# neuzxy/Distributed-TF-Serving

Hardware: AMD Instinct MI355X
Metric: CTR scores/sec (whole node) (higher is better)
Workload: dtype bf16; 1 GPU; model=deepfm (1Mx64 emb, 43 fields, MLP 1024-512-256), global_batch=16384, request_rows=512, parallelism=candidate-dp1 (one GPU, no fan-out), encoding=raw, aux_lane_cus=0

## Files before the change

### csrc/bindings_hip.cpp

```cpp
#include <torch/extension.h>

#include <cstring>

#include <ATen/hip/HIPContext.h>
#include <c10/core/DeviceGuard.h>
#include <c10/hip/HIPStream.h>

#include "kernels/launchers.h"
#include "comm/rccl_comm.h"
#include "live_bindings.h"
#include "runtime/numa.h"
#include "runtime/step_runner.h"

namespace {

hipStream_t cur_stream(const torch::Tensor& t) { return c10::hip::getCurrentHIPStream(t.device().index()).stream(); }

void check_hip(hipError_t e, const char* what) {
  TORCH_CHECK(e == hipSuccess, what, " failed: ", hipGetErrorString(e));
}

void check_dev(const torch::Tensor& t, const char* name) {
  TORCH_CHECK(t.is_cuda(), name, " must be a GPU tensor");
  TORCH_CHECK(t.is_contiguous(), name, " must be contiguous");
// ... 1183 lines not shown
                  reinterpret_cast<uintptr_t>(X.data_ptr()) % 16 == 0,
              "X needs unit column stride and 16-byte aligned rows");
  TORCH_CHECK(W2p.scalar_type() == torch::kFloat8_e4m3fn && W3p.scalar_type() == torch::kFloat8_e4m3fn,
              "W2p, W3p must be e4m3 (pack_bfrag_fp8)");
  TORCH_CHECK(W2p.numel() == N2 * K1 && W3p.numel() == N3 * N2, "packed weight sizes: 512 x 1024 and 256 x 512");
  for (auto* t : {&sw2, &b2, &sw3, &b3, &hw})
    TORCH_CHECK(t->scalar_type() == torch::kFloat32, "sw2, b2, sw3, b3, hw must be fp32");
  TORCH_CHECK(sw2.numel() == N2 && b2.numel() == N2, "sw2, b2 must have 512 elements");
  TORCH_CHECK(sw3.numel() == N3 && b3.numel() == N3 && hw.numel() == N3, "sw3, b3, hw must have 256 elements");
  TORCH_CHECK((act2 == 0 || act2 == 1) && (act3 == 0 || act3 == 1), "act must be 0 (none) or 1 (relu)");
  if (extra) {
    check_gpu(*extra, "extra");
    check_same_dev(X, *extra, "extra");
    check_extra(*extra, M);
  }
  if (out && out->is_cuda()) check_same_dev(X, *out, "out");
  c10::DeviceGuard g(X.device());
  torch::Tensor y;
  float* yp = score_out(X, M, out, y);
  check_hip(dtfs::launch_mlp_tail_fp8(X.data_ptr(), M <= 1 ? K1 : X.stride(0), int(M), int(K1), W2p.data_ptr(),
                                      sw2.data_ptr<float>(), b2.data_ptr<float>(), int(act2), int(N2), W3p.data_ptr(),
                                      sw3.data_ptr<float>(), b3.data_ptr<float>(), int(act3), int(N3),
                                      hw.data_ptr<float>(), float(hbias),
                                      extra ? extra->data_ptr<float>() : nullptr, extra ? extra_rows(*extra) : 0,
                                      extra ? extra_stride(*extra) : 0, sigmoid ? 2 : 0, yp, cur_stream(X)),
            "mlp_tail_fp8");
  return y;
}

torch::Tensor gather_mlp(torch::Tensor table, c10::optional<torch::Tensor> lin, c10::optional<torch::Tensor> arena,
                         c10::optional<torch::Tensor> ids, c10::optional<torch::Tensor> wts, int64_t B, int64_t F,
                         int64_t modulo, double bias, torch::Tensor W1p, torch::Tensor b1, torch::Tensor W2p,
                         torch::Tensor b2, int64_t act2, torch::Tensor W3p, torch::Tensor b3, int64_t act3,
                         torch::Tensor hw, double hbias, bool fm, bool sigmoid, c10::optional<torch::Tensor> out) {
  check_dev(table, "table");
  for (auto* t : {&W1p, &b1, &W2p, &b2, &W3p, &b3, &hw}) {
    check_dev(*t, "gather_mlp operand");
    check_same_dev(table, *t, "gather_mlp operand");
  }
  TORCH_CHECK(table.scalar_type() == torch::kBFloat16 && table.dim() == 2 && table.size(1) == 64 &&
                  table.is_contiguous(),
              "gather_mlp: table must be contiguous bf16 [V, 64]");
  const int64_t V = table.size(0);
  TORCH_CHECK(F >= 1 && F <= 64, "gather_mlp handles 1..64 fields");
  TORCH_CHECK(modulo > 0, "modulo must be positive");
  for (auto* t : {&W1p, &W2p, &W3p})
    TORCH_CHECK(t->scalar_type() == torch::kBFloat16 && t->is_contiguous(), "W1p / W2p / W3p: contiguous bf16 (pack_frag32)");
  TORCH_CHECK(b1.scalar_type() == torch::kFloat32 && b1.numel() == 1024 && b2.scalar_type() == torch::kFloat32 &&
                  b2.numel() == 512 && b3.scalar_type() == torch::kFloat32 && b3.numel() == 256 &&
                  hw.scalar_type() == torch::kFloat32 && hw.numel() == 256,
              "gather_mlp covers 64F -> 1024 -> 512 -> 256 -> 1 (fp32 biases / head weights)");
  TORCH_CHECK(W1p.numel() == 1024 * 64 * F && W2p.numel() == 512 * 1024 && W3p.numel() == 256 * 512,
              "packed weight sizes");
  TORCH_CHECK((act2 == 0 || act2 == 1) && (act3 == 0 || act3 == 1), "act must be 0 (none) or 1 (relu)");
  TORCH_CHECK(B >= 0 && B < (int64_t(1) << 31), "gather_mlp: row count");
  if (lin) {
    check_dev(*lin, "lin");
    TORCH_CHECK(lin->scalar_type() == torch::kFloat32 && lin->numel() == V, "lin must be fp32 [V]");
  }
  TORCH_CHECK(dtfs::gather_mlp_ok((B + 63) / 64 * 64, 1024, int(64 * F), 512, 256, int(F), V),
              "gather_mlp: shape outside the kernel's range");
  dtfs::EmbedArgs a;
  embed_gemm_inputs(table, arena, ids, wts, B, F, a);
  a.table = table.data_ptr();
  a.lin = lin ? lin->data_ptr<float>() : nullptr;
  a.B = int(B);
  a.F = int(F);
  a.D = 64;
  a.V = V;
  a.modulo = modulo;
  a.bias = float(bias);
  c10::DeviceGuard g(table.device());
  torch::Tensor y;
  float* yp = score_out(table, B, out, y);
  if (B == 0) return y;
  check_hip(dtfs::launch_gather_mlp(a, W1p.data_ptr(), b1.data_ptr<float>(), W2p.data_ptr(), b2.data_ptr<float>(),
                                    int(act2), W3p.data_ptr(), b3.data_ptr<float>(), int(act3), hw.data_ptr<float>(),
                                    float(hbias), fm, sigmoid ? 2 : 0, yp, cur_stream(table)),
            "gather_mlp");
  return y;
}

void unpack_arena(torch::Tensor arena, torch::Tensor packed, int64_t fields, int64_t narrow_modulo) {
  check_dev(arena, "arena");
  check_dev(packed, "packed");
  check_same_dev(arena, packed, "packed");
  TORCH_CHECK(arena.scalar_type() == torch::kUInt8 && arena.numel() > dtfs::kArenaPayloadOff, "arena: uint8 [cap]");
  TORCH_CHECK(packed.scalar_type() == torch::kInt64 && packed.dim() == 2, "packed must be int64 [B, W]");
  TORCH_CHECK(packed.size(1) * 8 >= (narrow_modulo > 0 ? 8 : 12) * fields, "packed rows too narrow for the field count");
  TORCH_CHECK(narrow_modulo >= 0 && narrow_modulo < (int64_t(1) << 31), "narrow_modulo must fit int32 rows");
  c10::DeviceGuard g(arena.device());
  check_hip(dtfs::launch_unpack_arena(arena.data_ptr(), packed.data_ptr<int64_t>(), int(packed.size(0)), int(fields),
                                      int(packed.size(1)), dtfs::kArenaMaxRequests, cur_stream(arena), narrow_modulo),
            "unpack_arena");
}

void arena_varint_decode(torch::Tensor arena, int64_t blocks) {
  check_dev(arena, "arena");
  TORCH_CHECK(arena.scalar_type() == torch::kUInt8 && arena.numel() > dtfs::kArenaPayloadOff, "arena: uint8 [cap]");
  c10::DeviceGuard g(arena.device());
  check_hip(dtfs::launch_arena_varint(arena.data_ptr(), int(blocks), cur_stream(arena)), "arena_varint_decode");
}

void pull_host(torch::Tensor dst, torch::Tensor src, int64_t nbytes, int64_t blocks) {
  check_dev(dst, "dst");
  TORCH_CHECK(src.device().is_cpu() && src.is_pinned(), "src must be pinned host memory");
  TORCH_CHECK(nbytes >= 0 && nbytes <= dst.nbytes() && nbytes <= src.nbytes(), "nbytes out of range");
  c10::DeviceGuard g(dst.device());
  check_hip(dtfs::launch_pull_host(dst.data_ptr(), src.data_ptr(), nbytes, int(blocks), cur_stream(dst)), "pull_host");
}

// ... 627 lines not shown
        py::arg("ring") = py::none(), py::arg("ring_ctr") = py::none(), py::arg("sample_every") = 0,
        py::arg("out_cols") = 0,
        "K1 + K5 with the rows read where they live (peer stores over xGMI, replica cache first)");
  m.def("peer_bag", &peer_bag, py::arg("ids"), py::arg("wts"), py::arg("arena"), py::arg("B"), py::arg("col0"),
        py::arg("hot"), py::arg("cbase"), py::arg("towner"), py::arg("toff"), py::arg("trows"), py::arg("tremote"),
        py::arg("chunk_shift"), py::arg("cache") = py::none(), py::arg("stats") = py::none(),
        py::arg("ring") = py::none(), py::arg("ring_ctr") = py::none(), py::arg("sample_every") = 0, py::arg("out"),
        "K1b multi-hot bags with the rows read where they live -> bf16 [B, T, 64]");
  m.def("peer_cache_fill", &peer_cache_fill, py::arg("keys"), py::arg("slots"), py::arg("cbase"), py::arg("towner"),
        py::arg("toff"), py::arg("trows"), py::arg("tremote"), py::arg("chunk_shift"), py::arg("rows"),
        "replica cache: copy the keys' table rows into their slots");
  m.def("device_alloc", &device_alloc, py::arg("nbytes"), py::arg("like"),
        "uint8 device buffer of exactly nbytes (its own hipMalloc allocation)");
  m.def("cache_index_build", &cache_index_build, py::arg("keys"), py::arg("slots"), py::arg("entries"),
        "replica cache: open-addressing index keys -> slots ({key, slot} entries pre-filled with -1)");
  m.def("ipc_export", &ipc_export, py::arg("t"), "(IPC handle bytes, byte offset) of a device tensor's allocation");
  m.def("ipc_open", &ipc_open, py::arg("handle"), py::arg("offset"), py::arg("shape"), py::arg("like"),
        "map a peer's ipc_export as a tensor (dtype / device of `like`)");
  m.def("head", &head, py::arg("x"), py::arg("w"), py::arg("bias") = 0.0, py::arg("extra") = py::none(),
        py::arg("sigmoid") = true);
  m.def("gemm_head", &gemm_head, py::arg("A"), py::arg("W"), py::arg("bias"), py::arg("act"), py::arg("hw"),
        py::arg("hbias") = 0.0, py::arg("extra") = py::none(), py::arg("sigmoid") = true, py::arg("out") = py::none());
  m.def("mlp_tail", &mlp_tail, py::arg("X"), py::arg("W2p"), py::arg("b2"), py::arg("act2"), py::arg("W3p"),
        py::arg("b3"), py::arg("act3"), py::arg("hw"), py::arg("hbias") = 0.0, py::arg("extra") = py::none(),
        py::arg("sigmoid") = true, py::arg("out") = py::none());
  m.def("mlp_tail_fp8", &mlp_tail_fp8, py::arg("X"), py::arg("W2p"), py::arg("sw2"), py::arg("b2"), py::arg("act2"),
        py::arg("W3p"), py::arg("sw3"), py::arg("b3"), py::arg("act3"), py::arg("hw"), py::arg("hbias") = 0.0,
        py::arg("extra") = py::none(), py::arg("sigmoid") = true, py::arg("out") = py::none(),
        "MX-fp8 two-layer MLP tail + head in one launch, operands quantised in-kernel (mlp_tail_fp8.hip)");
  m.def("gather_mlp", &gather_mlp, py::arg("table"), py::arg("lin"), py::arg("arena"), py::arg("ids"),
        py::arg("wts"), py::arg("B"), py::arg("F"), py::arg("modulo"), py::arg("bias"), py::arg("W1p"), py::arg("b1"),
        py::arg("W2p"), py::arg("b2"), py::arg("act2"), py::arg("W3p"), py::arg("b3"), py::arg("act3"), py::arg("hw"),
        py::arg("hbias"), py::arg("fm"), py::arg("sigmoid") = true, py::arg("out") = py::none(),
        "DeepFM / Wide&Deep tower in one launch: resolve + gather + FM + 3 MLP layers + head (gather_mlp.hip)");
  m.def("set_embed_wave_cap", &dtfs::set_embed_wave_cap, py::arg("waves"), py::arg("rows_in_flight") = 1,
        "pipelined embedding gather geometry: resident-wave cap (0 = one row per wave) and rows in flight per "
        "wave (1 or 2); tuning sweeps and tests");
  m.def("quant_rows_fp8", &quant_rows_fp8, py::arg("x"), py::arg("k_pad") = 1);
  m.def("dot_interaction_gather", &dot_interaction_gather, py::arg("dense"), py::arg("table"), py::arg("ids"),
        py::arg("modulo_f"), py::arg("offset_f"), py::arg("out_cols") = 0);
  m.def("bottom_mlp3", &bottom_mlp3, py::arg("wts"), py::arg("nd"), py::arg("W1"), py::arg("b1"), py::arg("W2"),
        py::arg("b2"), py::arg("W3"), py::arg("b3"));
  m.def("bottom_mlp3_arena", &bottom_mlp3_arena, py::arg("arena"), py::arg("B"), py::arg("nd"), py::arg("W1"),
        py::arg("b1"), py::arg("W2"), py::arg("b2"), py::arg("W3"), py::arg("b3"));
  m.def("dot_interaction_gather_arena", &dot_interaction_gather_arena, py::arg("dense"), py::arg("table"),
        py::arg("arena"), py::arg("id_col0"), py::arg("modulo_f"), py::arg("offset_f"), py::arg("out_cols") = 0);
  m.def("dot_interaction_gather_fp8", &dot_interaction_gather_fp8, py::arg("dense"), py::arg("emb_q"),
        py::arg("emb_scale"), py::arg("ids"), py::arg("modulo_f"), py::arg("offset_f"), py::arg("out_cols") = 0,
        "K1 + K5 on fp8 tables: e4m3 codes [V, 64] + one power-of-two scale per table (interaction_fp8.hip)");
  m.def("dot_interaction_gather_fp8_arena", &dot_interaction_gather_fp8_arena, py::arg("dense"), py::arg("emb_q"),
        py::arg("emb_scale"), py::arg("arena"), py::arg("id_col0"), py::arg("modulo_f"), py::arg("offset_f"),
        py::arg("out_cols") = 0);
  m.def("embedding_bag_fp8", &embedding_bag_fp8, py::arg("emb_q"), py::arg("emb_scale"), py::arg("indices"),
        py::arg("offsets"), py::arg("per_sample_weights") = py::none(), py::arg("modulo") = 0, py::arg("mean") = false,
        py::arg("out_bf16") = false, py::arg("out") = py::none(),
        "K1b on fp8 tables: bag b takes emb_scale[b % T]");
  m.def("cross_gemm_fp8", &cross_gemm_fp8, py::arg("q"), py::arg("sx"), py::arg("Wq"), py::arg("sw"), py::arg("bias"),
        py::arg("x0"), py::arg("xl"), py::arg("want_z") = true, py::arg("head_w") = py::none());
  m.def("cross_combine", &cross_combine, py::arg("y"), py::arg("x0"), py::arg("xl"), py::arg("want_z") = true,
        py::arg("k_pad") = 0, py::arg("head_w") = py::none(),
        "split DCN-v2 cross layer: z = x0*y + xl, optionally quantised (e4m3 + row scale) and/or dotted with head_w");
  m.def("unpack_arena", &unpack_arena, py::arg("arena"), py::arg("packed"), py::arg("fields"),
        py::arg("narrow_modulo") = 0);
  m.def("arena_varint_decode", &arena_varint_decode, py::arg("arena"), py::arg("blocks") = 256);
  m.def("pull_host", &pull_host, py::arg("dst"), py::arg("src"), py::arg("nbytes"), py::arg("blocks") = 128);
  m.def(
      "stream_write_u32",
// ... 269 lines not shown
```

### csrc/bindings_native.cpp

```cpp
#include <torch/extension.h>

#include <pybind11/stl.h>

#include <algorithm>
#include <cstring>

#include "runtime/batcher.h"
#include "runtime/arena.h"
#include "runtime/thread_pool.h"
#include "runtime/trace.h"
#include "wire/tensor_codec.h"
#include "live_bindings.h"
#include "runtime/narrow.h"
#include "net/hpack.h"
#include "runtime/numa.h"
#include "net/h2_client.h"

namespace py = pybind11;
using namespace dtfs;

namespace {

wire::DstType dst_type_of(const torch::Tensor& t) {
  switch (t.scalar_type()) {
// ... 245 lines not shown

void check_arena(const torch::Tensor& arena) {
  if (arena.device().type() != torch::kCPU || !arena.is_contiguous() || arena.scalar_type() != torch::kUInt8)
    throw py::value_error("arena must be a contiguous CPU uint8 tensor");
}

std::vector<std::pair<int64_t, int64_t>> arena_place(torch::Tensor arena, const std::vector<py::bytes>& reqs,
                                                     int64_t start) {
  check_arena(arena);
  std::vector<std::pair<const char*, size_t>> src(reqs.size());
  for (size_t i = 0; i < reqs.size(); ++i) {
    char* p;
    Py_ssize_t len;
    if (PyBytes_AsStringAndSize(reqs[i].ptr(), &p, &len) != 0) throw py::error_already_set();
    src[i] = {p, size_t(len)};
  }
  py::gil_scoped_release nogil;
  try {
    return runtime::arena_place(arena.data_ptr<uint8_t>(), arena.numel(), src, start);
  } catch (const std::invalid_argument& e) {
    py::gil_scoped_acquire g;
    throw py::value_error(e.what());
  }
}

ArenaBatch arena_build(torch::Tensor arena, const std::vector<std::pair<int64_t, int64_t>>& spans,
                       const std::string& ids_key, const std::string& wts_key, int64_t fields, int64_t max_rows,
                       int64_t varint_chunks, int64_t n_ranked, const std::vector<int32_t>& topk) {
  check_arena(arena);
  py::gil_scoped_release nogil;
  try {
    return runtime::arena_build(arena.data_ptr<uint8_t>(), arena.numel(), spans, ids_key, wts_key, fields, max_rows,
                                varint_chunks, n_ranked, topk);
  } catch (const std::invalid_argument& e) {
    py::gil_scoped_acquire g;
    throw py::value_error(e.what());
  }
}

void arena_unpack_cpu(torch::Tensor arena, torch::Tensor packed, int64_t fields) {
  check_arena(arena);
  if (packed.scalar_type() != torch::kInt64 || packed.dim() != 2 || !packed.is_contiguous())
    throw py::value_error("packed must be a contiguous int64 [B, W] tensor");
  if (packed.size(1) * 8 < 12 * fields) throw py::value_error("packed rows too narrow for the field count");
  const uint8_t* base = arena.data_ptr<uint8_t>();
  uint8_t* dst = reinterpret_cast<uint8_t*>(packed.data_ptr<int64_t>());
  const int64_t W = packed.size(1), B = packed.size(0);
  py::gil_scoped_release nogil;
  runtime::arena_unpack_cpu(base, dst, B, W, fields);
}

std::vector<py::bytes> encode_batch_responses(const std::string& name, const std::string& sig, py::object version,
                                              const std::string& key, torch::Tensor scores,
                                              const std::vector<int64_t>& rows, const std::vector<int64_t>& offsets,
                                              bool raw) {
  if (scores.device().type() != torch::kCPU || scores.scalar_type() != torch::kFloat32 || !scores.is_contiguous())
    throw py::value_error("scores must be a contiguous CPU fp32 tensor");
  if (rows.size() != offsets.size()) throw py::value_error("rows/offsets length mismatch");
  wire::ModelSpecOut spec;
  spec.name = name;
  spec.signature_name = sig;
  if (!version.is_none()) {
    spec.has_version = true;
    spec.version = version.cast<int64_t>();
  }
  const float* s = scores.data_ptr<float>();
// ... 308 lines not shown

  py::class_<ParsedBatch, std::shared_ptr<ParsedBatch>>(m, "ParsedBatch")
      .def_readonly("rows", &ParsedBatch::rows)
      .def_readonly("offsets", &ParsedBatch::offsets)
      .def_readonly("errors", &ParsedBatch::errors)
      .def_readonly("total_rows", &ParsedBatch::total_rows)
      .def_readonly("fields", &ParsedBatch::fields)
      .def("__len__", [](const ParsedBatch& b) { return b.views.size(); })
      .def("model_name", [](const ParsedBatch& b, size_t i) { return b.views.at(i).model_name; })
      .def("signature_name", [](const ParsedBatch& b, size_t i) { return b.views.at(i).signature_name; })
      .def("version", [](const ParsedBatch& b, size_t i) -> py::object {
        const auto& v = b.views.at(i);
        return v.has_version ? py::object(py::int_(v.version)) : py::object(py::none());
      })
      .def("output_filter", [](const ParsedBatch& b, size_t i) { return b.views.at(i).output_filter; })
      .def("decode", &decode_batch_range, py::arg("ids_dst"), py::arg("wts_dst"), py::arg("begin") = 0,
           py::arg("end") = int64_t(1) << 62, py::arg("base_row") = 0, py::arg("id_modulo") = 0);

  py::class_<ArenaBatch>(m, "ArenaBatch")
      .def_readonly("rows", &ArenaBatch::rows)
      .def_readonly("offsets", &ArenaBatch::offsets)
      .def_readonly("errors", &ArenaBatch::errors)
      .def_readonly("total_rows", &ArenaBatch::total_rows)
      .def_readonly("used_bytes", &ArenaBatch::used_bytes)
      .def_readonly("n_valid", &ArenaBatch::n_valid)
      .def_readonly("n_decoded", &ArenaBatch::n_decoded)
      .def_readonly("n_gpu_varint", &ArenaBatch::n_gpu_varint);
  m.attr("ARENA_PAYLOAD_OFF") = kArenaPayloadOff;
  m.attr("ARENA_MAX_REQUESTS") = kArenaMaxRequests;
  m.def("arena_place", &arena_place, py::arg("arena"), py::arg("requests"), py::arg("start") = 0);
  m.def("arena_build", &arena_build, py::arg("arena"), py::arg("spans"), py::arg("ids_key") = "feat_ids",
        py::arg("wts_key") = "feat_wts", py::arg("fields") = 43, py::arg("max_rows") = int64_t(1) << 40,
        py::arg("varint_chunks") = 0, py::arg("n_ranked") = 0, py::arg("topk") = std::vector<int32_t>());
  m.def("arena_varint_capacity", &runtime::arena_varint_capacity, py::arg("max_rows"), py::arg("fields"),
        py::arg("max_requests") = runtime::kArenaMaxRequests);
  m.def("arena_unpack_cpu", &arena_unpack_cpu, py::arg("arena"), py::arg("packed"), py::arg("fields"));

  m.def("parse_batch", &parse_batch, py::arg("requests"), py::arg("ids_key") = "feat_ids",
        py::arg("wts_key") = "feat_wts", py::arg("fields") = 43,
        "Parse many serialized PredictRequests (GIL released); see ParsedBatch.decode.");
  m.def("encode_batch_responses", &encode_batch_responses, py::arg("model_name"), py::arg("signature_name"),
        py::arg("version"), py::arg("key"), py::arg("scores"), py::arg("rows"), py::arg("offsets"),
        py::arg("raw") = false);

  m.def(
      "encode_predict_response",
      [](const std::string& name, const std::string& sig, py::object version,
         const std::vector<std::pair<std::string, torch::Tensor>>& outputs, bool raw) {
        std::vector<torch::Tensor> keep;
        auto outs = tensors_out(outputs, raw, &keep);
        auto spec = spec_of(name, sig, version);
        std::string s;
        {
          py::gil_scoped_release nogil;
          s = wire::encode_predict_response(spec, outs);
        }
        return py::bytes(s);
      },
      py::arg("model_name"), py::arg("signature_name"), py::arg("version"), py::arg("outputs"),
      py::arg("raw") = false);

  m.def(
      "encode_predict_request",
      [](const std::string& name, const std::string& sig, py::object version,
         const std::vector<std::pair<std::string, torch::Tensor>>& inputs, bool raw,
         const std::vector<std::string>& output_filter) {
// ... 106 lines not shown
```

### csrc/kernels/common.h

```cpp
#pragma once

#include <hip/hip_runtime.h>
#include <stdint.h>

namespace dtfs {
namespace kern {

typedef __bf16 bf16;
typedef __bf16 bf16x8 __attribute__((ext_vector_type(8)));
typedef __bf16 bf16x4 __attribute__((ext_vector_type(4)));
typedef float f32x4 __attribute__((ext_vector_type(4)));
typedef float f32x16 __attribute__((ext_vector_type(16)));
typedef int i32x4 __attribute__((ext_vector_type(4)));

constexpr int kWave = 64;

__device__ __forceinline__ float bf2f(bf16 x) { return float(x); }
__device__ __forceinline__ bf16 f2bf(float x) { return (bf16)x; }

__device__ __forceinline__ float wave_sum(float v) {
#pragma unroll
  for (int o = 32; o > 0; o >>= 1) v += __shfl_xor(v, o, 64);
  return v;
}
// ... 77 lines not shown

__device__ __forceinline__ ArenaRow arena_row_at(const uint8_t* payload, int2 o, int wcols, int idb) {
  ArenaRow r{payload + (o.x & 0x7fffffff), payload + (uint32_t(o.y) & kWtsOffMask), o.x < 0, kArenaAllWeights, 4};
  if (r.narrow) {
    r.wcols = wcols;
    r.idb = idb;
    r.wkind = int(uint32_t(o.y) >> 30);
  }
  return r;
}

__device__ __forceinline__ ArenaRow arena_row(const uint8_t* arena, int64_t payload_off, int64_t r) {
  const int64_t total = *reinterpret_cast<const int64_t*>(arena + 8);
  ArenaRow out{nullptr, nullptr, false, kArenaAllWeights, 4};
  if (r < total) {
    const uint8_t* payload = arena + payload_off;
    const int64_t rt = *reinterpret_cast<const int64_t*>(arena + 16);
    const int2 o = reinterpret_cast<const int2*>(payload + rt)[r];
    out = arena_row_at(payload, o, arena_narrow_wcols(arena), arena_narrow_idb(arena));
  }
  return out;
}

__device__ __forceinline__ void arena_feature(const ArenaRow& ar, int f, int64_t& id, float& w) {
  if (ar.narrow) {
    id = arena_narrow_id(ar, f);
    w = arena_narrow_w(ar, f);
  } else {
    id = int64_t(load_u64_unaligned(ar.ids + 8 * f));
    w = __uint_as_float(load_u32_unaligned(ar.wts + 4 * f));
  }
}

__device__ __forceinline__ int xcd_remap(int orig, int nwg) {
  constexpr int NX = 8;
  if (nwg <= NX) return orig;
  const int q = nwg / NX, r = nwg % NX;
  const int xcd = orig % NX, slot = orig / NX;
  const int base = xcd < r ? xcd * (q + 1) : r * (q + 1) + (xcd - r) * q;
  return base + slot;
}

}
}
```

### csrc/kernels/gather_mlp.hip

```cpp
#include <utility>

#include "asm_io.h"
#include "common.h"
#include "launchers.h"

namespace dtfs {
namespace kern {

typedef __bf16 bf16x2 __attribute__((ext_vector_type(2)));
typedef float f32x2 __attribute__((ext_vector_type(2)));

#ifdef DTFS_GM_STAMPS
__device__ unsigned long long g_gm_stamps[1024][4][16];
#define GM_T(k)                                             \
  do {                                                      \
    if (t == gm_t) gm_s[k] = __builtin_amdgcn_s_memtime(); \
  } while (0)
#define GM_AT(k)                              \
  do {                                        \
    gm_s[k] = __builtin_amdgcn_s_memtime(); \
  } while (0)
#else
#define GM_T(k) \
  do {          \
// ... 73 lines not shown
    constexpr int off = (kt >> 1) * 256;
    hf[kt & 1][0][s] = ds_read16_at<off>(hbase + (hb0 ^ x));
    hf[kt & 1][1][s] = ds_read16_at<off>(hbase + (hb1 ^ x));
  };
  gm_sfor<4>([&](auto S) { issue(std::integral_constant<int, 0>{}, S); });
  gm_sfor<NK>([&](auto KT) {
    constexpr int kt = decltype(KT)::value, b = kt & 1;
    gm_sfor<4>([&](auto S) {
      constexpr int s = decltype(S)::value;
      constexpr bool more = kt + 1 < NK;
      constexpr int nv = NJ * (3 - s) + (more ? NJ * s : 0);
      constexpr int nl = 2 * (3 - s) + (more ? 2 * s : 0);
      if constexpr (NJ == 4)
        wait_vm_4<nv>(wf[b][0][s], wf[b][1][s], wf[b][2][s], wf[b][3][s]);
      else
        wait_vm_2<nv>(wf[b][0][s], wf[b][1][s]);
      wait_lgkm2<nl>(hf[b][0][s], hf[b][1][s]);
#pragma unroll
      for (int jn = 0; jn < NJ; ++jn)
#pragma unroll
        for (int im = 0; im < 2; ++im)
          acc[jn][im] = __builtin_amdgcn_mfma_f32_32x32x16_bf16(wf[b][jn][s], hf[b][im][s], acc[jn][im], 0, 0, 0);
      if constexpr (more) issue(std::integral_constant<int, kt + 1>{}, S);
      __builtin_amdgcn_sched_barrier(0);
    });
  });
}

template <bool FM>
__global__ void __launch_bounds__(256, 1)
    gather_mlp_kernel(EmbedArgs ea, uint64_t magic, int F, const bf16x8* __restrict__ W1p,
                      const float* __restrict__ b1, const bf16x8* __restrict__ W2p, const float* __restrict__ b2,
                      int act2, const bf16x8* __restrict__ W3p, const float* __restrict__ b3, int act3,
                      const float* __restrict__ hw, float hbias, int M, int out_act, float* __restrict__ y) {
  constexpr int BM = 64;
  constexpr int N1 = 1024, N2 = 512, N3 = 256;
  constexpr int NS = 4;
  constexpr int SLOT = BM * 128;
  constexpr int FMAX = 64;
  constexpr int TROWS = NS * SLOT, TWTS = TROWS + FMAX * BM * 4;
  constexpr int H1P = N1 * 2, H2P = N2 * 2;
  constexpr int HOFF = BM * H1P;
  constexpr int BOFF = HOFF + 4 * BM * 4 + 2 * BM * 4;
  constexpr int SMEM = BOFF + (N1 + N2 + N3 + N3) * 4;
  static_assert(TWTS + FMAX * BM * 4 <= HOFF, "the K loop's ring and row tables live inside the h1 tile");
  const uint8_t* const table = static_cast<const uint8_t*>(ea.table);
  const int Vm1 = int(ea.V - 1);
#ifdef DTFS_GM_STAMPS
  unsigned long long gm_s[16] = {};
  const int gm_t = F / 2;
#endif
  GM_AT(0);
  __shared__ __attribute__((aligned(16))) uint8_t smem[SMEM];
  int32_t* const rows_l = reinterpret_cast<int32_t*>(smem + TROWS);
  float* const wts_l = reinterpret_cast<float*>(smem + TWTS);
  float* const red = reinterpret_cast<float*>(smem + HOFF);
  float* const fmv = red + 4 * BM;
  float* const firstv = fmv + BM;
  float* const b1s = reinterpret_cast<float*>(smem + BOFF);
  float* const b2s = b1s + N1;
  float* const b3s = b2s + N2;
  float* const hws = b3s + N3;
  const uint32_t aring_lds = lds_addr(smem);
  const uint32_t rows_lds = lds_addr(rows_l), wts_lds = lds_addr(wts_l);

  const int m0 = xcd_remap(blockIdx.x, gridDim.x) * BM;
  const int T = threadIdx.x;
  const int lane = T & 63;
  const int w = __builtin_amdgcn_readfirstlane(T >> 6);
  const int r32 = lane & 31, h = lane >> 5;

  const int arow0 = 16 * w + (lane >> 3);
  const int a_src = ((lane & 7) ^ ((lane >> 3) & 7)) << 4;
  const uint32_t aring_w = aring_lds + 16 * w * 128;
  const uint32_t idx_off = 4 * arow0;
  int aidx[2];
  auto read_idx = [&](int u) {
    const uint32_t base = rows_lds + min(u, F - 1) * (BM * 4) + idx_off;
// ... 61 lines not shown
#pragma unroll
      for (int g = 0; g < 16; ++g) acc[jn][im][g] = 0.f;
  auto mfma1 = [&](int jn, int im, int s) {
    acc[jn][im] = __builtin_amdgcn_mfma_f32_32x32x16_bf16(wf[jn][s], xf[im][s], acc[jn][im], 0, 0, 0);
  };
  auto pair = [&](int st, int k) {
    mfma1(2 * st + (k & 1), 0, k >> 1);
    mfma1(2 * st + (k & 1), 1, k >> 1);
  };
  auto fence = [] { __builtin_amdgcn_sched_barrier(0); };
  auto barrier = [] {
    __builtin_amdgcn_s_barrier();
    asm volatile("" ::: "memory");
  };
  auto wait_idx = [&] { asm volatile("s_waitcnt lgkmcnt(0)" : "+v"(aidx[0]), "+v"(aidx[1])::"memory"); };
#define WAIT_XS(N, s) wait_lgkm2<N>(xf[0][s], xf[1][s])

  auto vm_op = [&](int t, int g, int i) {
    if (g == 3) {
      load_w1(t, 6 + (i & 1), i >> 1);
    } else if (i < 8) {
      load_w1(t + 1, 2 * g + (i & 1), i >> 1);
    } else {
      stage_a(t + 3, g);
    }
  };

  reinterpret_cast<f32x4*>(b1s)[T] = reinterpret_cast<const f32x4*>(b1)[T];
  if (T < N2 / 4) reinterpret_cast<f32x4*>(b2s)[T] = reinterpret_cast<const f32x4*>(b2)[T];
  if (T < N3 / 4) {
    reinterpret_cast<f32x4*>(b3s)[T] = reinterpret_cast<const f32x4*>(b3)[T];
    reinterpret_cast<f32x4*>(hws)[T] = reinterpret_cast<const f32x4*>(hw)[T];
  }
#pragma unroll
  for (int g = 0; g < 3; ++g)
#pragma unroll
    for (int i = 0; i < 8; ++i) vm_op(-1, g, i);
  {
    constexpr int KR = FMAX / 4;
    const int rr = T & 63, f0 = T >> 6;
    const int b = m0 + rr;
    ArenaRow ar{nullptr, nullptr, false, kArenaAllWeights, 4};
    if (ea.arena && b < ea.B) ar = arena_row(static_cast<const uint8_t*>(ea.arena), kArenaPayloadOff, b);
    int64_t id[KR];
    float wv[KR];
#pragma unroll
    for (int k = 0; k < KR; ++k) {
      const int f = f0 + 4 * k;
      id[k] = 0;
      wv[k] = 0.f;
      if (f < F && b < ea.B) {
        if (ea.arena) {
          if (ar.ids) arena_feature(ar, f, id[k], wv[k]);
        } else {
          id[k] = ea.ids64 ? static_cast<const int64_t*>(ea.ids)[int64_t(b) * ea.ids_ld + f]
                           : int64_t(static_cast<const int32_t*>(ea.ids)[int64_t(b) * ea.ids_ld + f]);
          wv[k] = !ea.wts ? 1.f
                  : ea.wts16 ? __uint_as_float(uint32_t(static_cast<const uint16_t*>(ea.wts)[int64_t(b) * ea.wts_ld + f]) << 16)
                             : static_cast<const float*>(ea.wts)[int64_t(b) * ea.wts_ld + f];
        }
      }
    }
    float lsum = 0.f;
#pragma unroll
    for (int k = 0; k < KR; ++k) {
      const int f = f0 + 4 * k;
      if (f < F) {
        int64_t g = magic ? hash_row_magic(id[k], ea.modulo, magic) : hash_row(id[k], ea.modulo);
        g = g < 0 ? 0 : (g > Vm1 ? Vm1 : g);
        rows_l[f * BM + rr] = int32_t(g);
        wts_l[f * BM + rr] = wv[k];
        if (ea.lin) lsum += ea.lin[g] * wv[k];
      }
    }
    red[f0 * BM + rr] = lsum;
  }
  __syncthreads();
  if (T < BM) firstv[T] = ea.bias + red[T] + red[BM + T] + red[2 * BM + T] + red[3 * BM + T];
  read_idx(0);
  wait_idx();
  stage_a(0, 0);
  stage_a(0, 1);
  read_idx(1);
  wait_idx();
  stage_a(1, 0);
  stage_a(1, 1);
  read_idx(2);
  wait_idx();
  stage_a(2, 0);
  stage_a(2, 1);
  asm volatile("s_waitcnt vmcnt(2)" ::: "memory");
  barrier();
  scale_read(0);
  scale_wait();
#pragma unroll
  for (int q = 0; q < 2; ++q)
#pragma unroll
    for (int p = 0; p < 4; ++p) scale_pair(0, q, p);
  read_idx(3);
  wait_idx();
  barrier();
  read_xs(0, 0);
  read_xs(0, 1);
  read_xs(0, 2);
  GM_AT(1);

#pragma unroll 1
  for (int t = 0; t < F; ++t) {
    if constexpr (FM) {
      if (t == F - 1) {
#pragma unroll
        for (int a = 0; a < 2; ++a) {
          float part = -fsq[a];
#pragma unroll
          for (int d = 0; d < 8; ++d) part += fs[a][d] * fs[a][d];
          part += __shfl_xor(part, 1, 64);
          part += __shfl_xor(part, 2, 64);
          part += __shfl_xor(part, 4, 64);
          if (sc_c == 0) fmv[sc_r0 + 32 * a] = 0.5f * part;
        }
        __builtin_amdgcn_s_waitcnt(0xc07f);
      }
    }
    wait_vm8<18>(wf[0], wf[1]);
    GM_T(2);
// ... 163 lines not shown
#pragma unroll
    for (int im = 0; im < 2; ++im) {
      const float v = part[im] + __shfl_xor(part[im], 32, 64);
      if (he == 0) red[w * BM + 32 * im + r32e] = v;
    }
  }
  __syncthreads();
  if (tid_e < BM) {
    const int m = m0 + tid_e;
    if (m < M) {
      float s = hbias + firstv[tid_e];
      if constexpr (FM) s += fmv[tid_e];
#pragma unroll
      for (int ww = 0; ww < 4; ++ww) s += red[ww * BM + tid_e];
      y[m] = out_act == 2 ? sigmoidf(s) : s;
    }
  }
#ifdef DTFS_GM_STAMPS
  GM_AT(12);
  if (lane_e == 0 && blockIdx.x < 1024)
    for (int k = 0; k < 13; ++k) g_gm_stamps[blockIdx.x][w][k] = gm_s[k];
#endif
}

}

bool gather_mlp_ok(int64_t Mp, int N1, int K1, int N2, int N3, int F, int64_t V) {
  return N1 == 1024 && N2 == 512 && N3 == 256 && K1 == 64 * F && Mp % 64 == 0 && F >= 1 && F <= 64 && V >= 1 &&
         V <= (int64_t(1) << 25);
}

hipError_t launch_gather_mlp(const EmbedArgs& a, const void* W1p, const float* b1, const void* W2p, const float* b2,
                             int act2, const void* W3p, const float* b3, int act3, const float* hw, float hbias,
                             bool fm, int out_act, float* y, hipStream_t st) {
  if (a.B == 0) return hipSuccess;
  const int64_t Mp = (int64_t(a.B) + 63) / 64 * 64;
  if (!gather_mlp_ok(Mp, 1024, 64 * a.F, 512, 256, a.F, a.V) || a.B < 0 || a.modulo <= 0 || !a.table ||
      (!a.arena && !a.ids) || a.modulo_f || a.shard_lo_f || !W1p || !b1 || !W2p || !b2 || !W3p || !b3 || !hw || !y)
    return hipErrorInvalidValue;
  const uint64_t magic = a.modulo < (int64_t(1) << 32) ? ~uint64_t(0) / uint64_t(a.modulo) : 0;
  const int grid = int(Mp / 64);
  if (fm)
    hipLaunchKernelGGL((kern::gather_mlp_kernel<true>), dim3(grid), dim3(256), 0, st, a, magic, a.F,
                       static_cast<const kern::bf16x8*>(W1p), b1, static_cast<const kern::bf16x8*>(W2p), b2, act2,
                       static_cast<const kern::bf16x8*>(W3p), b3, act3, hw, hbias, a.B, out_act, y);
  else
    hipLaunchKernelGGL((kern::gather_mlp_kernel<false>), dim3(grid), dim3(256), 0, st, a, magic, a.F,
                       static_cast<const kern::bf16x8*>(W1p), b1, static_cast<const kern::bf16x8*>(W2p), b2, act2,
                       static_cast<const kern::bf16x8*>(W3p), b3, act3, hw, hbias, a.B, out_act, y);
  return hipGetLastError();
}

}
```

### csrc/kernels/launchers.h

```cpp
#pragma once

#include <hip/hip_runtime.h>
#include <stdint.h>

namespace dtfs {

hipError_t launch_pack_ids(const void* ids, bool ids64, int32_t* out, int64_t n, int F, const int64_t* modulo_f,
                           const int64_t* offset_f, int64_t modulo, hipStream_t st);

struct RouteArgs {
  const void* ids = nullptr;
  bool ids64 = true;
  int64_t ld = 0;
  const uint8_t* arena = nullptr;
  const float* wts = nullptr;
  int64_t wts_ld = 0;
  int B = 0, F = 0, W = 1, tm = 1, hot = 1;
  const int32_t* col = nullptr;
  const int64_t* mod = nullptr;
  const int64_t* off = nullptr;
  int32_t* out = nullptr;
  float* out_w = nullptr;
};
hipError_t launch_shard_route(const RouteArgs& a, hipStream_t st);
// ... 57 lines not shown
};

hipError_t launch_gemm_gather(const void* table, int64_t V, const int32_t* rows_t, const float* wts_t, int64_t Mp,
                              int F, const void* W, const float* bias, void* C, int64_t ldc, float* fm_part, int M,
                              int N, int epi, hipStream_t st, const float* cross_w = nullptr,
                              const float* cross_c = nullptr, int cross_n = 0);

bool gemm_gather1w_ok(int64_t Mp, int N, int F, bool cross, int64_t V);
hipError_t launch_gemm_gather1w(const void* table, int64_t V, const int32_t* rows_t, const float* wts_t, int64_t Mp,
                                int F, const void* Wp, const float* bias, void* C, int64_t ldc, float* fm_part, int M,
                                int N, int epi, hipStream_t st);

hipError_t launch_gemm(const void* A, int64_t lda, const void* W, int64_t ldw, const float* bias, const float* sa,
                       const float* sw, void* C, int64_t ldc, bool out_f32, const void* X0, const void* XL,
                       int64_t ldx, int M, int N, int K, int epi, bool fp8, hipStream_t st,
                       int variant = 0, const MxIO* mx = nullptr);

hipError_t launch_gemm_head(const void* A, int64_t lda, const void* W, int64_t ldw, const float* bias, int act,
                            const float* hw, float hbias, const float* extra, int out_act, float* y, int M, int N,
                            int K, hipStream_t st, int extra_n = 1, int64_t extra_ld = 0);

hipError_t launch_mlp_tail(const void* X, int64_t ldx, int M, int K1, const void* W2p, const float* b2, int act2,
                           int N2, const void* W3p, const float* b3, int act3, int N3, const float* hw, float hbias,
                           const float* extra, int extra_n, int64_t extra_ld, int out_act, float* y, hipStream_t st);

hipError_t launch_mlp_tail_fp8(const void* X, int64_t ldx, int M, int K1, const void* W2p, const float* sw2,
                               const float* b2, int act2, int N2, const void* W3p, const float* sw3, const float* b3,
                               int act3, int N3, const float* hw, float hbias, const float* extra, int extra_n,
                               int64_t extra_ld, int out_act, float* y, hipStream_t st);

bool gather_mlp_ok(int64_t Mp, int N1, int K1, int N2, int N3, int F, int64_t V);
hipError_t launch_gather_mlp(const EmbedArgs& a, const void* W1p, const float* b1, const void* W2p, const float* b2,
                             int act2, const void* W3p, const float* b3, int act3, const float* hw, float hbias,
                             bool fm, int out_act, float* y, hipStream_t st);

hipError_t launch_cross_v1(const void* x0, int64_t ldx, int B, int d, int L, const float* w, const float* b,
                           void* out_x, int64_t ldo, const float* head_w, float* out_dot, hipStream_t st);

hipError_t launch_dot_interaction(const void* dense, int64_t ldd, const void* emb, int T, int B, void* out,
                                  int64_t ldo, int out_cols, hipStream_t st, const int64_t* emb_off = nullptr,
                                  const int64_t* emb_stride = nullptr, int64_t emb_rows = 0);

hipError_t launch_dense_pad(const float* x, int64_t ldx, int M, int n, void* y, int K, hipStream_t st);

hipError_t launch_head(const void* x, int64_t ldx, const float* w, float bias, const float* extra, int M, int K,
                       int act, float* out, hipStream_t st, int extra_n = 1, int64_t extra_ld = 0);

hipError_t launch_quant_rows_fp8(const void* x, int64_t ldx, int M, int K, void* q, int64_t ldq, float* scale,
                                 hipStream_t st, int Kq = 0);

hipError_t launch_cross_combine(const void* y, const void* x0, const void* xl, int64_t ld, int M, int N, void* z,
                                int64_t ldz, void* q, int64_t ldq, float* scale, int Kq, const float* head_w,
                                float* dot, hipStream_t st);

struct CrossGemmArgs {
  const void* A = nullptr;
  int64_t lda = 0;
  const void* W = nullptr;
  int64_t ldw = 0;
  const float* bias = nullptr;
  const float* sa = nullptr;
  const float* sw = nullptr;
  void* Z = nullptr;
  int64_t ldz = 0;
  const void* X0 = nullptr;
  const void* XL = nullptr;
  int64_t ldx = 0;
// ... 72 lines not shown
```

### distributed_tf_serving_amd/serving/arena.py

```python
from __future__ import annotations

from dataclasses import dataclass
from typing import List, Sequence, Tuple

import torch

from ..ops import native


@dataclass(frozen=True)
class ArenaLayout:
    fields: int
    max_rows: int
    max_requests: int = 1024
    gpu_varint: bool = True

    @property
    def varint_chunks(self) -> int:
        if not self.gpu_varint:
            return 0
        return native().arena_varint_capacity(self.max_rows, self.fields, self.max_requests)

    @property
    def varint_blocks(self) -> int:
        return min(1024, self.varint_chunks)

    def decode_varints(self, arena_dev: torch.Tensor) -> None:
        if self.gpu_varint:
            from ..ops import hip

            hip().arena_varint_decode(arena_dev, self.varint_blocks)

    @property
    def payload_off(self) -> int:
        return native().ARENA_PAYLOAD_OFF

    @property
    def capacity(self) -> int:
        per_row = 28 * self.fields + 8
        return (self.payload_off + self.max_rows * per_row + self.max_requests * 1024 + 128
                + 32 * self.varint_chunks)

    def alloc(self, device="cpu", pin: bool = False) -> torch.Tensor:
        return torch.zeros(self.capacity, dtype=torch.uint8, device=device, pin_memory=pin)

    def place(self, arena: torch.Tensor, requests: Sequence[bytes], start: int = 0) -> List[Tuple[int, int]]:
        return native().arena_place(arena, list(requests), start)

    def build(self, arena: torch.Tensor, spans: Sequence[Tuple[int, int]], ids_key="feat_ids", wts_key="feat_wts",
              n_ranked: int = 0, topk: Sequence[int] = ()):
        return native().arena_build(arena, list(spans), ids_key, wts_key, self.fields, self.max_rows,
                                    self.varint_chunks, int(n_ranked), [int(k) for k in topk])

    def unpack_cpu(self, arena: torch.Tensor, packed: torch.Tensor) -> torch.Tensor:
        native().arena_unpack_cpu(arena, packed, self.fields)
        return packed
```

Baseline: 152.0 million scores/s.

## Stage contiguous arena tile ids/weights into LDS with bulk vector loads in gather_mlp

When the 64 rows of a tile come from one contiguous narrow-arena run, the kernel detects this once per tile. It bulk-copies the whole id and weight block into shared memory with 16-byte loads and decodes each row's ids and weights from LDS, replacing per-row, per-feature arena resolution. The linear-term loads are issued asynchronously and consumed after the first A-tile staging, overlapping them with the pipeline prologue. This adds a fast-path detection check, extra LDS use inside the h1 region and more code complexity, and falls back to the old per-row path otherwise.

```diff
diff --git a/csrc/bindings_hip.cpp b/csrc/bindings_hip.cpp
--- a/csrc/bindings_hip.cpp
+++ b/csrc/bindings_hip.cpp
@@ -1239,7 +1239,8 @@
                          c10::optional<torch::Tensor> ids, c10::optional<torch::Tensor> wts, int64_t B, int64_t F,
                          int64_t modulo, double bias, torch::Tensor W1p, torch::Tensor b1, torch::Tensor W2p,
                          torch::Tensor b2, int64_t act2, torch::Tensor W3p, torch::Tensor b3, int64_t act3,
-                         torch::Tensor hw, double hbias, bool fm, bool sigmoid, c10::optional<torch::Tensor> out) {
+                         torch::Tensor hw, double hbias, bool fm, bool sigmoid, c10::optional<torch::Tensor> out,
+                         bool staged) {
   check_dev(table, "table");
   for (auto* t : {&W1p, &b1, &W2p, &b2, &W3p, &b3, &hw}) {
     check_dev(*t, "gather_mlp operand");
@@ -1283,7 +1284,7 @@
   if (B == 0) return y;
   check_hip(dtfs::launch_gather_mlp(a, W1p.data_ptr(), b1.data_ptr<float>(), W2p.data_ptr(), b2.data_ptr<float>(),
                                     int(act2), W3p.data_ptr(), b3.data_ptr<float>(), int(act3), hw.data_ptr<float>(),
-                                    float(hbias), fm, sigmoid ? 2 : 0, yp, cur_stream(table)),
+                                    float(hbias), fm, sigmoid ? 2 : 0, yp, cur_stream(table), staged),
             "gather_mlp");
   return y;
 }
@@ -1977,7 +1978,9 @@
         py::arg("wts"), py::arg("B"), py::arg("F"), py::arg("modulo"), py::arg("bias"), py::arg("W1p"), py::arg("b1"),
         py::arg("W2p"), py::arg("b2"), py::arg("act2"), py::arg("W3p"), py::arg("b3"), py::arg("act3"), py::arg("hw"),
         py::arg("hbias"), py::arg("fm"), py::arg("sigmoid") = true, py::arg("out") = py::none(),
-        "DeepFM / Wide&Deep tower in one launch: resolve + gather + FM + 3 MLP layers + head (gather_mlp.hip)");
+        py::arg("staged") = true,
+        "DeepFM / Wide&Deep tower in one launch: resolve + gather + FM + 3 MLP layers + head (gather_mlp.hip). "
+        "staged=False forces the per-feature resolve on every tile (tests, A/B runs)");
   m.def("set_embed_wave_cap", &dtfs::set_embed_wave_cap, py::arg("waves"), py::arg("rows_in_flight") = 1,
         "pipelined embedding gather geometry: resident-wave cap (0 = one row per wave) and rows in flight per "
         "wave (1 or 2); tuning sweeps and tests");
diff --git a/csrc/bindings_native.cpp b/csrc/bindings_native.cpp
--- a/csrc/bindings_native.cpp
+++ b/csrc/bindings_native.cpp
@@ -301,6 +301,27 @@
   try {
     return runtime::arena_build(arena.data_ptr<uint8_t>(), arena.numel(), spans, ids_key, wts_key, fields, max_rows,
                                 varint_chunks, n_ranked, topk);
+  } catch (const std::invalid_argument& e) {
+    py::gil_scoped_acquire g;
+    throw py::value_error(e.what());
+  }
+}
+
+ArenaBatch arena_build_narrow(torch::Tensor arena, const std::vector<std::tuple<int64_t, int64_t, int64_t, int>>& reqs,
+                              int64_t fields, int64_t max_rows, int64_t narrow_wcols, int64_t narrow_id_bytes) {
+  check_arena(arena);
+  std::vector<runtime::ArenaItem> items(reqs.size());
+  for (size_t i = 0; i < reqs.size(); ++i) {
+    items[i].narrow = true;
+    items[i].rows = std::get<0>(reqs[i]);
+    items[i].ids_off = std::get<1>(reqs[i]);
+    items[i].wts_off = std::get<2>(reqs[i]);
+    items[i].wkind = std::get<3>(reqs[i]);
+  }
+  py::gil_scoped_release nogil;
+  try {
+    return runtime::arena_build_items(arena.data_ptr<uint8_t>(), arena.numel(), items, "feat_ids", "feat_wts", fields,
+                                      max_rows, 0, narrow_wcols, narrow_id_bytes);
   } catch (const std::invalid_argument& e) {
     py::gil_scoped_acquire g;
     throw py::value_error(e.what());
@@ -675,6 +696,8 @@
   m.def("arena_build", &arena_build, py::arg("arena"), py::arg("spans"), py::arg("ids_key") = "feat_ids",
         py::arg("wts_key") = "feat_wts", py::arg("fields") = 43, py::arg("max_rows") = int64_t(1) << 40,
         py::arg("varint_chunks") = 0, py::arg("n_ranked") = 0, py::arg("topk") = std::vector<int32_t>());
+  m.def("arena_build_narrow", &arena_build_narrow, py::arg("arena"), py::arg("requests"), py::arg("fields") = 43,
+        py::arg("max_rows") = int64_t(1) << 40, py::arg("narrow_wcols") = 0, py::arg("narrow_id_bytes") = 4);
   m.def("arena_varint_capacity", &runtime::arena_varint_capacity, py::arg("max_rows"), py::arg("fields"),
         py::arg("max_requests") = runtime::kArenaMaxRequests);
   m.def("arena_unpack_cpu", &arena_unpack_cpu, py::arg("arena"), py::arg("packed"), py::arg("fields"));
diff --git a/csrc/kernels/common.h b/csrc/kernels/common.h
--- a/csrc/kernels/common.h
+++ b/csrc/kernels/common.h
@@ -133,6 +133,42 @@
   }
 }
 
+struct ArenaTileRun {
+  bool ok = false;
+  int n = 0;
+  int idb = 4;
+  int wcols = 0;
+  int wkind = kWtsF32;
+  uint32_t ids_off = 0;
+  uint32_t wts_off = 0;
+};
+
+__device__ __forceinline__ int wts_kind_bytes(int wkind) { return wkind == kWtsF32 ? 4 : (wkind == kWtsBf16 ? 2 : 0); }
+
+__device__ __forceinline__ ArenaTileRun arena_tile_run(const uint8_t* arena, int64_t payload_off, int64_t m0,
+                                                       int64_t rows_B, int F, int lane) {
+  ArenaTileRun t;
+  const int64_t total = *reinterpret_cast<const int64_t*>(arena + 8);
+  const int64_t rt = *reinterpret_cast<const int64_t*>(arena + 16);
+  const int hw = *reinterpret_cast<const int32_t*>(arena + 36);
+  const int64_t live = (rows_B < total ? rows_B : total) - m0;
+  t.n = int(live < 0 ? 0 : (live > 64 ? 64 : live));
+  t.idb = arena_narrow_idb(arena);
+  t.wcols = hw > 0 && hw < F ? hw : F;
+  if (t.n == 0) return t;
+  int2 o = make_int2(0, 0);
+  if (lane < t.n) o = reinterpret_cast<const int2*>(arena + payload_off + rt)[m0 + lane];
+  const int o0x = __builtin_amdgcn_readfirstlane(o.x), o0y = __builtin_amdgcn_readfirstlane(o.y);
+  t.wkind = int(uint32_t(o0y) >> 30);
+  t.ids_off = uint32_t(o0x) & 0x7fffffffu;
+  t.wts_off = uint32_t(o0y) & kWtsOffMask;
+  const uint32_t istride = uint32_t(F * t.idb), wstride = uint32_t(t.wcols * wts_kind_bytes(t.wkind));
+  const bool mine = lane >= t.n || (uint32_t(o.x) == uint32_t(o0x) + uint32_t(lane) * istride &&
+                                    uint32_t(o.y) == uint32_t(o0y) + uint32_t(lane) * wstride);
+  t.ok = o0x < 0 && t.wkind <= kWtsOnes && __all(mine);
+  return t;
+}
+
 __device__ __forceinline__ int xcd_remap(int orig, int nwg) {
   constexpr int NX = 8;
   if (nwg <= NX) return orig;
diff --git a/csrc/kernels/gather_mlp.hip b/csrc/kernels/gather_mlp.hip
--- a/csrc/kernels/gather_mlp.hip
+++ b/csrc/kernels/gather_mlp.hip
@@ -129,7 +129,8 @@
     gather_mlp_kernel(EmbedArgs ea, uint64_t magic, int F, const bf16x8* __restrict__ W1p,
                       const float* __restrict__ b1, const bf16x8* __restrict__ W2p, const float* __restrict__ b2,
                       int act2, const bf16x8* __restrict__ W3p, const float* __restrict__ b3, int act3,
-                      const float* __restrict__ hw, float hbias, int M, int out_act, float* __restrict__ y) {
+                      const float* __restrict__ hw, float hbias, int M, int out_act, int staged_ok,
+                      float* __restrict__ y) {
   constexpr int BM = 64;
   constexpr int N1 = 1024, N2 = 512, N3 = 256;
   constexpr int NS = 4;
@@ -141,6 +142,9 @@
   constexpr int BOFF = HOFF + 4 * BM * 4 + 2 * BM * 4;
   constexpr int SMEM = BOFF + (N1 + N2 + N3 + N3) * 4;
   static_assert(TWTS + FMAX * BM * 4 <= HOFF, "the K loop's ring and row tables live inside the h1 tile");
+  constexpr int SRUN = (BM * FMAX * 4 + 15 + 15) / 16 * 16;
+  constexpr int SIDS = TWTS + FMAX * BM * 4, SWTS = SIDS + SRUN + 16;
+  static_assert(SIDS == 64 * 1024 && SWTS + SRUN <= HOFF, "the staging buffers live inside the h1 tile");
   const uint8_t* const table = static_cast<const uint8_t*>(ea.table);
   const int Vm1 = int(ea.V - 1);
 #ifdef DTFS_GM_STAMPS
@@ -268,18 +272,109 @@
     reinterpret_cast<f32x4*>(b3s)[T] = reinterpret_cast<const f32x4*>(b3)[T];
     reinterpret_cast<f32x4*>(hws)[T] = reinterpret_cast<const f32x4*>(hw)[T];
   }
+  constexpr int KR = FMAX / 4;
+  const int rr = lane, f0 = w;
+  const uint8_t* const arena = static_cast<const uint8_t*>(ea.arena);
+  ArenaTileRun run;
+  if (arena && staged_ok && (reinterpret_cast<uintptr_t>(arena) & 15) == 0)
+    run = arena_tile_run(arena, kArenaPayloadOff, m0, ea.B, F, lane);
+  const bool staged = __builtin_amdgcn_readfirstlane(int(run.ok)) != 0;
+  uint32_t skew_i = 0, skew_w = 0;
+  constexpr int NB = 5;
+  i32x4 bulk[NB];
+  const i32x4 *src_i = nullptr, *src_w = nullptr;
+  int nci = 0, ntot = 0;
+  auto bulk_load = [&](int c0) {
+#pragma unroll
+    for (int j = 0; j < NB; ++j) {
+      const int c = c0 + j * 256;
+      if (c < ntot) bulk[j] = c < nci ? src_i[c] : src_w[c - nci];
+    }
+  };
+  auto bulk_store = [&](int c0) {
+#pragma unroll
+    for (int j = 0; j < NB; ++j) {
+      const int c = c0 + j * 256;
+      if (c < ntot) *reinterpret_cast<i32x4*>(smem + (c < nci ? SIDS + 16 * c : SWTS + 16 * (c - nci))) = bulk[j];
+    }
+  };
+  if (staged) {
+    const uint8_t* const ip = arena + kArenaPayloadOff + run.ids_off;
+    const uint8_t* const wp = arena + kArenaPayloadOff + run.wts_off;
+    skew_i = uint32_t(reinterpret_cast<uintptr_t>(ip) & 15);
+    skew_w = uint32_t(reinterpret_cast<uintptr_t>(wp) & 15);
+    src_i = reinterpret_cast<const i32x4*>(ip - skew_i);
+    src_w = reinterpret_cast<const i32x4*>(wp - skew_w);
+    nci = int(skew_i + uint32_t(run.n * F * run.idb) + 15) >> 4;
+    const int nbw = run.n * run.wcols * wts_kind_bytes(run.wkind);
+    ntot = nci + (nbw ? int(skew_w + uint32_t(nbw) + 15) >> 4 : 0);
+    bulk_load(T);
+  }
 #pragma unroll
   for (int g = 0; g < 3; ++g)
 #pragma unroll
     for (int i = 0; i < 8; ++i) vm_op(-1, g, i);
-  {
-    constexpr int KR = FMAX / 4;
-    const int rr = T & 63, f0 = T >> 6;
+  float wv[KR], lv[KR] = {};
+  float lsum = 0.f;
+  if (staged) {
+    bulk_store(T);
+    if (ntot > NB * 256) {
+      bulk_load(T + NB * 256);
+      bulk_store(T + NB * 256);
+    }
+    __syncthreads();
+    const int idb = run.idb, wbytes = wts_kind_bytes(run.wkind);
+    const uint32_t ib = SIDS + skew_i + uint32_t(rr * F * idb);
+    const uint32_t wb = SWTS + skew_w + uint32_t(rr * run.wcols * wbytes);
+    const uint32_t idmask = idb == 3 ? 0xffffffu : 0xffffffffu;
+    const uint32_t w16 = run.wkind == kWtsBf16 ? 16u : 0u;
+    const uint32_t wand = run.wkind == kWtsOnes ? 0u : 0xffffffffu, wor = run.wkind == kWtsOnes ? 0x3f800000u : 0u;
+    uint32_t d0[KR], d1[KR], dw[KR];
+#pragma unroll
+    for (int k = 0; k < KR; ++k) {
+      const uint32_t ia = ib + uint32_t(idb * (f0 + 4 * k)), wa = wb + uint32_t(wbytes * (f0 + 4 * k));
+      d0[k] = *reinterpret_cast<const uint32_t*>(smem + (ia & ~3u));
+      d1[k] = *reinterpret_cast<const uint32_t*>(smem + (ia & ~3u) + 4);
+      dw[k] = *reinterpret_cast<const uint32_t*>(smem + (wa & ~3u));
+    }
+    int32_t id[KR];
+    bool in = true;
+#pragma unroll
+    for (int k = 0; k < KR; ++k) {
+      const int f = f0 + 4 * k;
+      const uint32_t ia = ib + uint32_t(idb * f), wa = wb + uint32_t(wbytes * f);
+      const uint32_t v = __builtin_amdgcn_alignbyte(d1[k], d0[k], ia & 3) & idmask;
+      const uint32_t wbits = (((dw[k] >> ((wa & 2) * 8 & w16)) << w16) & wand) | wor;
+      const bool on = f < F && rr < run.n;
+      id[k] = on ? int32_t(v) : 0;
+      wv[k] = on && f < run.wcols ? __uint_as_float(wbits) : 0.f;
+      in = in && id[k] >= 0 && int64_t(id[k]) < ea.modulo;
+    }
+    if (__builtin_amdgcn_readfirstlane(__all(in)) == 0) {
+#pragma unroll
+      for (int k = 0; k < KR; ++k)
+        id[k] = int32_t(magic ? hash_row_magic(id[k], ea.modulo, magic) : hash_row(id[k], ea.modulo));
+    }
+    uint32_t lo[KR], prev = uint32_t(min(rr, Vm1)) * 4u;
+#pragma unroll
+    for (int k = 0; k < KR; ++k) {
+      const int f = f0 + 4 * k;
+      if (f < F) {
+        const int g = min(max(id[k], 0), Vm1);
+        rows_l[f * BM + rr] = g;
+        wts_l[f * BM + rr] = wv[k];
+        prev = uint32_t(g) * 4u;
+      }
+      lo[k] = prev;
+    }
+    const void* const lbase = ea.lin ? static_cast<const void*>(ea.lin) : ea.table;
+#pragma unroll
+    for (int k = 0; k < KR; ++k) asm volatile("global_load_dword %0, %1, %2" : "=v"(lv[k]) : "v"(lo[k]), "s"(lbase));
+  } else {
     const int b = m0 + rr;
     ArenaRow ar{nullptr, nullptr, false, kArenaAllWeights, 4};
     if (ea.arena && b < ea.B) ar = arena_row(static_cast<const uint8_t*>(ea.arena), kArenaPayloadOff, b);
     int64_t id[KR];
-    float wv[KR];
 #pragma unroll
     for (int k = 0; k < KR; ++k) {
       const int f = f0 + 4 * k;
@@ -297,7 +392,6 @@
         }
       }
     }
-    float lsum = 0.f;
 #pragma unroll
     for (int k = 0; k < KR; ++k) {
       const int f = f0 + 4 * k;
@@ -309,10 +403,9 @@
         if (ea.lin) lsum += ea.lin[g] * wv[k];
       }
     }
-    red[f0 * BM + rr] = lsum;
-  }
-  __syncthreads();
-  if (T < BM) firstv[T] = ea.bias + red[T] + red[BM + T] + red[2 * BM + T] + red[3 * BM + T];
+  }
+  asm volatile("s_waitcnt lgkmcnt(0)" ::: "memory");
+  barrier();
   read_idx(0);
   wait_idx();
   stage_a(0, 0);
@@ -325,8 +418,19 @@
   wait_idx();
   stage_a(2, 0);
   stage_a(2, 1);
-  asm volatile("s_waitcnt vmcnt(2)" ::: "memory");
+  asm volatile("s_waitcnt vmcnt(2)"
+               : "+v"(lv[0]), "+v"(lv[1]), "+v"(lv[2]), "+v"(lv[3]), "+v"(lv[4]), "+v"(lv[5]), "+v"(lv[6]), "+v"(lv[7]),
+                 "+v"(lv[8]), "+v"(lv[9]), "+v"(lv[10]), "+v"(lv[11]), "+v"(lv[12]), "+v"(lv[13]), "+v"(lv[14]),
+                 "+v"(lv[15])::"memory");
+  if (staged && ea.lin) {
+#pragma unroll
+    for (int k = 0; k < KR; ++k)
+      if (f0 + 4 * k < F) lsum += lv[k] * wv[k];
+  }
+  red[f0 * BM + rr] = lsum;
+  asm volatile("s_waitcnt lgkmcnt(0)" ::: "memory");
   barrier();
+  if (T < BM) firstv[T] = ea.bias + red[T] + red[BM + T] + red[2 * BM + T] + red[3 * BM + T];
   scale_read(0);
   scale_wait();
 #pragma unroll
@@ -556,7 +660,7 @@
 
 hipError_t launch_gather_mlp(const EmbedArgs& a, const void* W1p, const float* b1, const void* W2p, const float* b2,
                              int act2, const void* W3p, const float* b3, int act3, const float* hw, float hbias,
-                             bool fm, int out_act, float* y, hipStream_t st) {
+                             bool fm, int out_act, float* y, hipStream_t st, bool staged) {
   if (a.B == 0) return hipSuccess;
   const int64_t Mp = (int64_t(a.B) + 63) / 64 * 64;
   if (!gather_mlp_ok(Mp, 1024, 64 * a.F, 512, 256, a.F, a.V) || a.B < 0 || a.modulo <= 0 || !a.table ||
@@ -567,11 +671,11 @@
   if (fm)
     hipLaunchKernelGGL((kern::gather_mlp_kernel<true>), dim3(grid), dim3(256), 0, st, a, magic, a.F,
                        static_cast<const kern::bf16x8*>(W1p), b1, static_cast<const kern::bf16x8*>(W2p), b2, act2,
-                       static_cast<const kern::bf16x8*>(W3p), b3, act3, hw, hbias, a.B, out_act, y);
+                       static_cast<const kern::bf16x8*>(W3p), b3, act3, hw, hbias, a.B, out_act, int(staged), y);
   else
     hipLaunchKernelGGL((kern::gather_mlp_kernel<false>), dim3(grid), dim3(256), 0, st, a, magic, a.F,
                        static_cast<const kern::bf16x8*>(W1p), b1, static_cast<const kern::bf16x8*>(W2p), b2, act2,
-                       static_cast<const kern::bf16x8*>(W3p), b3, act3, hw, hbias, a.B, out_act, y);
+                       static_cast<const kern::bf16x8*>(W3p), b3, act3, hw, hbias, a.B, out_act, int(staged), y);
   return hipGetLastError();
 }
 
diff --git a/csrc/kernels/launchers.h b/csrc/kernels/launchers.h
--- a/csrc/kernels/launchers.h
+++ b/csrc/kernels/launchers.h
@@ -113,7 +113,7 @@
 bool gather_mlp_ok(int64_t Mp, int N1, int K1, int N2, int N3, int F, int64_t V);
 hipError_t launch_gather_mlp(const EmbedArgs& a, const void* W1p, const float* b1, const void* W2p, const float* b2,
                              int act2, const void* W3p, const float* b3, int act3, const float* hw, float hbias,
-                             bool fm, int out_act, float* y, hipStream_t st);
+                             bool fm, int out_act, float* y, hipStream_t st, bool staged = true);
 
 hipError_t launch_cross_v1(const void* x0, int64_t ldx, int B, int d, int L, const float* w, const float* b,
                            void* out_x, int64_t ldo, const float* head_w, float* out_dot, hipStream_t st);
diff --git a/distributed_tf_serving_amd/serving/arena.py b/distributed_tf_serving_amd/serving/arena.py
--- a/distributed_tf_serving_amd/serving/arena.py
+++ b/distributed_tf_serving_amd/serving/arena.py
@@ -55,3 +55,43 @@
     def unpack_cpu(self, arena: torch.Tensor, packed: torch.Tensor) -> torch.Tensor:
         native().arena_unpack_cpu(arena, packed, self.fields)
         return packed
+
+
+WTS_F32, WTS_BF16, WTS_ONES = 0, 1, 2
+
+
+def narrow_arena(requests, fields: int, modulo: int, id_bytes: int = 3, wcols: int = 0, offsets=None):
+    n = native()
+    wc = wcols if wcols > 0 else fields
+    wbytes = {WTS_F32: 4, WTS_BF16: 2, WTS_ONES: 0}
+    placed, cur = [], 0
+    for i, (ids, wts, kind) in enumerate(requests):
+        rows = ids.shape[0]
+        nib, nwb = rows * fields * id_bytes, rows * wc * wbytes[kind]
+        if offsets is not None:
+            io, wo = offsets[i]
+        else:
+            io = cur
+            wo = (io + nib + 4 + 3) & ~3
+            cur = (wo + nwb + 3) & ~3
+        placed.append((rows, io, wo, kind, nib, nwb))
+    end = max([max(io + nib + 4, wo + nwb) for _, io, wo, _, nib, nwb in placed] + [0])
+    total = sum(p[0] for p in placed)
+    arena = torch.zeros(n.ARENA_PAYLOAD_OFF + end + 8 * total + 256, dtype=torch.uint8)
+    pay = arena[n.ARENA_PAYLOAD_OFF:]
+    for (ids, wts, kind), (rows, io, wo, _, nib, nwb) in zip(requests, placed):
+        ids = ids.contiguous()
+        if id_bytes == 3:
+            pay[io:io + nib] = n.narrow_ids24(ids, modulo)
+        else:
+            pay[io:io + nib] = n.narrow_ids(ids, modulo).reshape(-1).view(torch.uint8)
+        w = wts[:, :wc].contiguous().float()
+        if kind == WTS_F32:
+            pay[wo:wo + nwb] = w.reshape(-1).view(torch.uint8)
+        elif kind == WTS_BF16:
+            assert torch.equal(w.to(torch.bfloat16).float(), w), "bf16 weights must be bf16 values"
+            pay[wo:wo + nwb] = w.to(torch.bfloat16).reshape(-1).view(torch.uint8)
+        else:
+            assert bool((w == 1).all()), "implicit weights must all be 1.0"
+    batch = n.arena_build_narrow(arena, [p[:4] for p in placed], fields, 1 << 40, wcols, id_bytes)
+    return arena[:batch.used_bytes].clone(), batch
```

After: 157.3 million scores/s (median of 6 runs). +3.5%, better.
